# Arbol-Project/dcdf

Hardware: AMD Instinct MI355X
Metric: raster cells/s encoded (Snapshot+Log build) (higher is better)
Workload: dtype int32; 1 GPU; configs[2]: 4096x4096x365 i32 raster, seed 0xDCDF0003, tiled into 3072 [<=32,256,256] chunks; 3072 of them on this GPU; workload_key=config2/i32/n3072/w1, chunks_total=3072, chunks_on_rank0=3072, cells_total=6123683840, k=2, device=gfx950:sramecc+:xnack- AMD Radeon Graphics, 256 CUs, failed_tiles_rank0=0, encoded_bytes_rank0=4115239087, snapshots_rank0=3072, bytes_verified_vs_oracle=0, parallelism=chunks sharded over 1 GPU(s), no data-path collective

## Files before the change

dcdf_amd/csrc/k2r_encode.h:

```cpp
#pragma once
#include "k2r_exec.h"


#ifndef K2R_DIAG_SKIP
#define K2R_DIAG_SKIP 0
#endif

namespace k2r {

template <int LOG2S>
struct EncCfg {
    static_assert(LOG2S >= 3 && LOG2S <= 8, "kernel body written for sidelen 8..256 (the library dispatches 16..256)");
    static constexpr int H = LOG2S;
    static constexpr int S = 1 << LOG2S;
    static constexpr int NBLK = 1 << (2 * (LOG2S - 3));
    static constexpr int NT = NBLK;
    static constexpr int NW = NT < 64 ? 1 : NT / 64;
    static constexpr int NTOP = ((1 << (2 * (H - 2))) - 1) / 3;
    static constexpr int NTOPX = NTOP - (1 << (2 * (H - 3)));
    static constexpr int TBW = (NTOPX + 31) / 32 + 1;
    static constexpr int MAXV = ((1 << (2 * (H + 1))) - 1) / 3;
    static constexpr int MAXT = ((1 << (2 * H)) - 1) / 3;
    static constexpr int WV = (MAXV + 31) / 32;
    static constexpr int WT = (MAXT + 31) / 32;
// ... 205 lines not shown
            const uint32_t ob = o << 3;
            const ll2 a = *(__attribute__((address_space(1))) const ll2*)((gptr)ib + ob);
            const ll2 b = *(__attribute__((address_space(1))) const ll2*)((gptr)ib + ob + 16);
            x[0] = a.x; x[1] = a.y; x[2] = b.x; x[3] = b.y;
#else
            for (int i = 0; i < 4; i++) x[i] = ib[o + i];
#endif
            if (VEC == 4) {
                const double f[4] = {as_f64(x[0]), as_f64(x[1]), as_f64(x[2]), as_f64(x[3])};
                int32_t v[4];
                fixed4_f64(f, ta, (double)((int64_t)1 << ta.fbits), v, err);
#pragma unroll
                for (int dc = 0; dc < 4; dc++) dst[cell_m(dr, dc)] = v[dc];
            } else {
#pragma unroll
                for (int dc = 0; dc < 4; dc++) {
                    bad |= (uint32_t)(((uint64_t)x[dc] + (uint64_t)VALUE_LIMIT) >> 31 != 0);
                    dst[cell_m(dr, dc)] = (int32_t)x[dc];
                }
            }
        }
        if (bad && err == 0) err = ERR_RANGE;
    } else if (VEC) {
        const int32_t* ib = (const int32_t*)ta.base + (int64_t)inst * ta.st;
        const uint32_t o0 = rj * (uint32_t)ta.sr + cj;
#pragma unroll
        for (int dr = 0; dr < 4; dr++) {
            const uint32_t o = o0 + (uint32_t)dr * (uint32_t)ta.sr;
            int32_t v[4];
#if defined(__HIP_DEVICE_COMPILE__)
            typedef __attribute__((address_space(1))) const char* gptr;
            const uint32_t ob = o << 2;
#ifdef K2R_NT_LOADS
            typedef int i4v __attribute__((ext_vector_type(4)));
            const i4v av = __builtin_nontemporal_load((__attribute__((address_space(1))) const i4v*)((gptr)ib + ob));
            const int4 a = {av.x, av.y, av.z, av.w};
#else
            const int4 a = *(__attribute__((address_space(1))) const int4*)((gptr)ib + ob);
#endif
            v[0] = a.x; v[1] = a.y; v[2] = a.z; v[3] = a.w;
#else
            for (int i = 0; i < 4; i++) v[i] = ib[o + i];
#endif
            if (VEC == 2) {
                const float f[4] = {as_f32(v[0]), as_f32(v[1]), as_f32(v[2]), as_f32(v[3])};
                fixed4_f32(f, ta, (float)((int64_t)1 << ta.fbits), v, err);
            }
#pragma unroll
            for (int dc = 0; dc < 4; dc++) dst[cell_m(dr, dc)] = v[dc];
        }
    } else {
#pragma unroll
        for (int m = 0; m < 16; m++) {
            uint32_t r = rj + m_dr(m), c = cj + m_dc(m);
            if (PADDED) {
                r = r < ta.rows ? r : ta.rows - 1;
                c = c < ta.cols ? c : ta.cols - 1;
            }
            int64_t off = (int64_t)inst * ta.st + (int64_t)r * ta.sr + (int64_t)c * ta.sc;
            dst[m] = narrow(load_stored(ta, off, err), err);
        }
    }
}

template <class C>
K2R_HD uint32_t compact_slot(int tid, int j) {
    return 4u * (uint32_t)tid + (uint32_t)j;
}
template <class C>
K2R_HD void load_compact_raw(const uint32_t* scmp, int tid, int j, uint32_t (&w)[8]) {
    const uint32_t* p = scmp + (size_t)compact_slot<C>(tid, j) * 8;
#if defined(__HIP_DEVICE_COMPILE__)
    typedef __attribute__((address_space(1))) const char* gptr;
    const uint32_t ob = compact_slot<C>(tid, j) * 32u;
    const uint4 a = *(__attribute__((address_space(1))) const uint4*)((gptr)scmp + ob);
    const uint4 b = *(__attribute__((address_space(1))) const uint4*)((gptr)scmp + ob + 16);
    (void)p;
    w[0] = a.x; w[1] = a.y; w[2] = a.z; w[3] = a.w;
    w[4] = b.x; w[5] = b.y; w[6] = b.z; w[7] = b.w;
#else
    for (int i = 0; i < 8; i++) w[i] = p[i];
#endif
}
template <class C>
K2R_HD void load_compact(const uint32_t* scmp, int tid, int j, int32_t base, int32_t (&dst)[16]) {
    uint32_t w[8];
    load_compact_raw<C>(scmp, tid, j, w);
#pragma unroll
    for (int p = 0; p < 2; p++)
#pragma unroll
        for (int c = 0; c < 4; c++) {
            dst[8 * p + c] = base + (int32_t)(w[4 * p + c] & 0xffffu);
            dst[8 * p + 4 + c] = base + (int32_t)(w[4 * p + c] >> 16);
        }
}
template <class C>
K2R_HD void store_compact(uint32_t* scmp, int tid, int j, int32_t base, const int32_t (&src)[16]) {
    uint32_t* p = scmp + (size_t)compact_slot<C>(tid, j) * 8;
    uint32_t w[8];
#pragma unroll
    for (int q = 0; q < 2; q++)
#pragma unroll
        for (int c = 0; c < 4; c++) w[4 * q + c] = (uint32_t)(src[8 * q + c] - base) | ((uint32_t)(src[8 * q + 4 + c] - base) << 16);
#if defined(__HIP_DEVICE_COMPILE__)
    *(__attribute__((address_space(1))) uint4*)p = uint4{w[0], w[1], w[2], w[3]};
    *(__attribute__((address_space(1))) uint4*)(p + 4) = uint4{w[4], w[5], w[6], w[7]};
#else
    for (int i = 0; i < 8; i++) p[i] = w[i];
#endif
}
K2R_HD uint32_t pk_min_u16(uint32_t a, uint32_t b) {
#if defined(__HIP_DEVICE_COMPILE__)
    typedef unsigned short u16x2 __attribute__((ext_vector_type(2)));
    return __builtin_bit_cast(uint32_t, __builtin_elementwise_min(__builtin_bit_cast(u16x2, a), __builtin_bit_cast(u16x2, b)));
#else
    const uint32_t lo = (a & 0xffffu) < (b & 0xffffu) ? (a & 0xffffu) : (b & 0xffffu), hi = (a >> 16) < (b >> 16) ? (a >> 16) : (b >> 16);
    return lo | (hi << 16);
#endif
}
K2R_HD uint32_t pk_max_u16(uint32_t a, uint32_t b) {
#if defined(__HIP_DEVICE_COMPILE__)
    typedef unsigned short u16x2 __attribute__((ext_vector_type(2)));
    return __builtin_bit_cast(uint32_t, __builtin_elementwise_max(__builtin_bit_cast(u16x2, a), __builtin_bit_cast(u16x2, b)));
#else
    const uint32_t lo = (a & 0xffffu) > (b & 0xffffu) ? (a & 0xffffu) : (b & 0xffffu), hi = (a >> 16) > (b >> 16) ? (a >> 16) : (b >> 16);
    return lo | (hi << 16);
#endif
}
K2R_HD uint32_t nz(uint32_t v) {
#if defined(__HIP_DEVICE_COMPILE__)
    uint32_t r;
    asm("v_min_u32 %0, 1, %1" : "=v"(r) : "v"(v));
    return r;
#else
    return v != 0 ? 1u : 0u;
#endif
}
K2R_HD uint32_t mul24(uint32_t a, uint32_t b) {
#if defined(__HIP_DEVICE_COMPILE__)
    return __umul24(a, b);
#else
    return a * b;
#endif
}
K2R_HD uint32_t pk_lo16(uint32_t lo, uint32_t hi) {
#if defined(__HIP_DEVICE_COMPILE__)
    return __builtin_amdgcn_perm(hi, lo, 0x05040100u);
#else
    return (lo & 0xffffu) | (hi << 16);
#endif
}

K2R_HD uint32_t opaque(uint32_t v) {
#if defined(__HIP_DEVICE_COMPILE__)
    asm volatile("" : "+v"(v));
#endif
    return v;
}

K2R_HD void sched_fence() {
#if defined(__HIP_DEVICE_COMPILE__) && !defined(K2R_NO_SCHED_FENCE)
    __builtin_amdgcn_sched_barrier(0);
#endif
}

template <bool PADDED, int VEC>
K2R_HD void load_quad(const TileArgs& ta, uint32_t inst, uint32_t rq, uint32_t cq, int32_t (&dst)[4], int32_t& err) {
    if (VEC == 3 || VEC == 4) {
        const int64_t* ib = (const int64_t*)ta.base + (int64_t)inst * ta.st;
        const uint32_t o0 = rq * (uint32_t)ta.sr + cq;
        uint32_t bad = 0;
        int64_t raw[4];
#pragma unroll
        for (int dr = 0; dr < 2; dr++) {
            const uint32_t o = o0 + (uint32_t)dr * (uint32_t)ta.sr;
            int64_t x0, x1;
#if defined(__HIP_DEVICE_COMPILE__)
            typedef __attribute__((address_space(1))) const char* gptr;
            typedef long long ll2 __attribute__((ext_vector_type(2)));
            const ll2 a = *(__attribute__((address_space(1))) const ll2*)((gptr)ib + (o << 3));
            x0 = a.x; x1 = a.y;
#else
            x0 = ib[o]; x1 = ib[o + 1];
#endif
            raw[2 * dr] = x0;
            raw[2 * dr + 1] = x1;
        }
        if (VEC == 4) {
            const double f[4] = {as_f64(raw[0]), as_f64(raw[1]), as_f64(raw[2]), as_f64(raw[3])};
            fixed4_f64(f, ta, (double)((int64_t)1 << ta.fbits), dst, err);
        } else {
#pragma unroll
// ... 1296 lines not shown
        auto log_vmin = [&](int h, uint32_t j) -> int32_t {
            const int a = C::top_off(h) + (int)j;
            return sh.tmin[a] - sh.smin[a];
        };

        auto top_decode = [&](uint32_t n, int& h, uint32_t& j) {
            h = 4;
#pragma unroll
            for (int k = 4; k < H; k++)
                if (n >= (uint32_t)(C::top_off(k + 1) - C::NBLK)) h = k + 1;
            j = n - (uint32_t)(C::top_off(h) - C::NBLK);
        };
        auto tbit = [&](int h, uint32_t j) -> uint32_t { return (uint32_t)(C::top_off(h) - C::NBLK) + j; };

        ex.par_nosync([&](int tid, EncRegs& r) {
            uint32_t sI3 = 0, lI3 = 0;
            uint32_t wide = (r.flags >> 28) & 1u;
            Cls lMax, lMin;
            uint32_t sTop = 0, lTop = 0;
            auto node = [&](int h, uint32_t j) {
                if (PS(h, j)) {
                    if (h == 3) sI3 = 1;
                    else {
                        ex.lds_or(&sh.tbS[tbit(h, j) >> 5], 1u << (tbit(h, j) & 31));
                        sTop += (uint32_t)packTop(h);
                    }
                }
                if (have_s) {
                    const bool visL = (h == H) ? true : PL(h + 1, j >> 2);
                    const bool pL = PL(h, j);
                    const int32_t vx = log_vmax(h, j), vn = log_vmin(h, j);
                    lMax.add1(vx, visL);
                    lMin.add1(vn, pL);
                    wide |= ((visL && (vx < -32768 || vx > 32767)) || (pL && (vn < -32768 || vn > 32767))) ? 1u : 0u;
                    if (pL) {
                        if (h == 3) lI3 = 1;
                        else {
                            ex.lds_or(&sh.tbL[tbit(h, j) >> 5], 1u << (tbit(h, j) & 31));
                            lTop += (uint32_t)packTop(h);
                        }
                    }
                }
            };
            const uint32_t wt = opaque((uint32_t)tid);
            node(3, wt);
            if (tid == 0) {
                sh.stI = 0;
                sh.stQ = 0;
            }
            if (wt < (uint32_t)C::NTOPX) {
                int h;
                uint32_t j;
                top_decode(wt, h, j);
                node(h, j);
            }
            r.sc[1] = sI3 | (lI3 << 16);
            r.sc[2] = sTop;
            r.sc[4] = lTop;
            r.sc[5] = lMax.c1 | (lMin.c1 << 16);
            r.sc[6] = wide;
            uint32_t cL0 = 0, cL1 = 0, mL1 = 0, cL2 = 0, mL2 = 0;
            if (have_s) {
                const uint32_t fl = sh.li[tid];
                cL0 = popc32(sh.lq[tid][0]) + popc32(sh.lq[tid][1]);
                cL1 = popc32(fl & 0x0f0f0f0fu);
                mL1 = popc32(fl & 0xf0f0f0f0u);
#pragma unroll
                for (int j = 0; j < 4; j++) {
                    const int32_t vx = rec16(r.d2[j] & 0xffffu), vn = rec16(r.d2[j] >> 16);
                    r.d2[j] = ((uint32_t)vx & 0xffffu) | ((uint32_t)vn << 16);
                    const bool P2L = ((r.u2 >> j) & 1u) == 0 && ((r.flags >> j) & 1u) == 0;
                    cL2 += lI3 ? lng(vx) : 0u;
                    mL2 += P2L ? lng(vn) : 0u;
                }
            }
            r.sc[7] = cL0;
            r.sc[8] = cL1 | (cL2 << 16);
            r.sc[9] = mL1 | (mL2 << 16);
        });
        ex.stamp(2);
        ex.template scan_begin<10>();
        ex.stamp(3);

        auto classes_pass = [&](const int which) {
#ifdef K2R_SIM_TRACE
            if (EX::kSim) __builtin_printf("classes_pass(%d) inst=%u\n", which, inst);
#endif
            ex.par_nosync([&](int tid, EncRegs& r) {
                uint32_t r0, c0;
                blk_origin(tid, r0, c0);
                int32_t lerr = 0;
                Cls vMax, vMin;
                auto cnode = [&](int h, uint32_t j) {
                    if (which == 0) {
                        vMax.add(zz32(snap_vmax(h, j)), (h == H) ? true : PS(h + 1, j >> 2));
                        vMin.add(zz32(snap_vmin(h, j)), PS(h, j));
                    } else {
                        vMax.add(zz32(log_vmax(h, j)), (h == H) ? true : PL(h + 1, j >> 2));
                        vMin.add(zz32(log_vmin(h, j)), PL(h, j));
                    }
                };
                cnode(3, (uint32_t)tid);
                if (tid < C::NTOPX) {
                    int h;
                    uint32_t j;
                    top_decode((uint32_t)tid, h, j);
                    cnode(h, j);
                }
                const int32_t mn3 = sh.tmin[tid], mx3 = sh.tmax[tid];
                const bool inv3 = inval(r0, c0);
                const bool P3 = !inv3 && mn3 != mx3 && (which == 0 || sh.eq[tid] == 0);
#pragma unroll 1
                for (int j = 0; j < 4; j++) {
                    const uint32_t rj = r0 + 4 * (j >> 1), cj = c0 + 4 * (j & 1);
                    const bool inv2 = inval(rj, cj);
                    int32_t t16[16], s16[16];
                    load_sub16<PADDED, VEC>(ta, inst, r0, c0, j, t16, lerr);
                    if (which != 0) load_sub16<PADDED, VEC>(ta, s_idx, r0, c0, j, s16, lerr);
                    int32_t mn2 = t16[0], mx2 = t16[0], smn2 = 0, smx2 = 0;
#pragma unroll
                    for (int i = 1; i < 16; i++) {
                        mn2 = t16[i] < mn2 ? t16[i] : mn2;
                        mx2 = t16[i] > mx2 ? t16[i] : mx2;
                    }
                    if (which != 0) {
                        smn2 = smx2 = s16[0];
#pragma unroll
                        for (int i = 1; i < 16; i++) {
                            smn2 = s16[i] < smn2 ? s16[i] : smn2;
                            smx2 = s16[i] > smx2 ? s16[i] : smx2;
                        }
                    }
                    const bool unif2 = inv2 || mn2 == mx2;
                    bool P2;
                    if (which == 0) {
                        P2 = !unif2;
                        vMax.add(zz32(inv2 ? mx3 : mx3 - mx2), P3);
                        vMin.add(zz32(mn2 - mn3), P2);
                    } else {
                        P2 = !unif2 && ((r.flags >> j) & 1u) == 0;
                        vMax.add(zz32(inv2 ? 0 : mx2 - smx2), P3);
                        vMin.add(zz32(mn2 - smn2), P2);
                    }
                    if (!P2) continue;
#pragma unroll
                    for (int qq = 0; qq < 4; qq++) {
                        const uint32_t rq = rj + 2 * (qq >> 1), cq = cj + 2 * (qq & 1);
                        const bool inv1 = inval(rq, cq);
                        const int32_t mn1 = min4(t16[4 * qq], t16[4 * qq + 1], t16[4 * qq + 2], t16[4 * qq + 3]);
                        const int32_t mx1 = max4(t16[4 * qq], t16[4 * qq + 1], t16[4 * qq + 2], t16[4 * qq + 3]);
                        const bool unif1 = inv1 || mn1 == mx1;
                        if (which == 0) {
                            vMax.add(zz32(inv1 ? mx2 : mx2 - mx1), true);
                            vMin.add(zz32(mn1 - mn2), !unif1);
#pragma unroll
                            for (int i = 0; i < 4; i++)
                                vMax.add(zz32(inval(rq + (i >> 1), cq + (i & 1)) ? mx1 : mx1 - t16[4 * qq + i]), !unif1);
                        } else {
                            int32_t d[4];
#pragma unroll
                            for (int i = 0; i < 4; i++)
                                d[i] = inval(rq + (i >> 1), cq + (i & 1)) ? 0 : t16[4 * qq + i] - s16[4 * qq + i];
                            const int32_t smn1 = min4(s16[4 * qq], s16[4 * qq + 1], s16[4 * qq + 2], s16[4 * qq + 3]);
                            const int32_t smx1 = max4(s16[4 * qq], s16[4 * qq + 1], s16[4 * qq + 2], s16[4 * qq + 3]);
                            const bool P1 = !unif1 && !(d[0] == d[1] && d[0] == d[2] && d[0] == d[3]);
                            vMax.add(zz32(inv1 ? 0 : mx1 - smx1), true);
                            vMin.add(zz32(mn1 - smn1), P1);
#pragma unroll
                            for (int i = 0; i < 4; i++) vMax.add(zz32(d[i]), P1);
                        }
                    }
                }
                r.sc[10] = vMax.c1;
                r.sc[11] = vMax.c2;
                r.sc[12] = vMax.c3;
                r.sc[13] = vMin.c1;
                r.sc[14] = vMin.c2;
                r.sc[15] = vMin.c3;
            });
            ex.template reduce<6, 10>();
        };

        const bool cap254 = have_s && (blk_count - 1 == 254);
        auto plan = [&](const int stage) {
            ex.par([&](int tid, EncRegs&) {
                uint32_t T10[10];
                if (stage == 1) {
                    ex.template scan_finish<10>(T10);
                    for (uint32_t w = (uint32_t)tid; w <= (uint32_t)C::WT; w += NT) {
                        sh.bmT[w] = 0;
                        sh.bmE[w] = 0;
                        sh.bmM[0][w] = 0;
                    }
                    for (uint32_t w = (uint32_t)tid; w <= (uint32_t)C::WV; w += NT) sh.bmV0[w] = 0;
                }
                constexpr bool kTwoLanes = !EX::kSim && NT >= 2;
                if (tid >= (stage == 1 && kTwoLanes ? 2 : 1)) return;
                auto& pl = sh.pl;
                auto choose = [&](bool snap, const Totals<C>& W, uint32_t size, uint32_t narrow) {
                    pl.as_snapshot = snap ? 1u : 0u;
                    pl.isize = size;
                    pl.use_stash = (!snap && narrow && 5u * stI + 3u * stQ <= stash_cap && stI == W.Ni[2] && stQ == W.Ni[1]) ? 1u : 0u;
                    uint32_t rr = 0;
#pragma unroll
                    for (int h = 4; h <= H; h++) {
                        sh.ttR[h] = rr;
                        rr += W.Ni[h];
                    }
                    sh.ttR[H + 1] = rr;
                };
                if (stage == 1) {
                    const uint32_t t0 = T10[0], t1 = T10[1], t2 = T10[2], t3 = T10[3], t4 = T10[4], t5 = T10[5], t6 = T10[6], t7 = T10[7],
                                   t8 = T10[8], t9 = T10[9];
                    const uint32_t narrow = (have_s && t6 == 0) ? 1u : 0u;
                    const uint32_t lv2 = t5 & 0xffffu, lv1 = lv2 + (t8 >> 16), lv0 = lv1 + (t8 & 0xffffu);
                    const uint32_t lm2 = t5 >> 16, lm1 = lm2 + (t9 >> 16);
                    auto cand = [&](uint32_t c, Totals<C>& T, DacLayout& V, DacLayout& M, uint32_t& eo) {
                        T.from(c == 0 ? ((uint64_t)t0 | ((uint64_t)(t1 & 0xffffu) << 30)) : ((uint64_t)t3 | ((uint64_t)(t1 >> 16) << 30)),
                               c == 0 ? t2 : t4);
                        eo = 13 + bitmap_size(T.LT);
                        const uint32_t vbase = c == 0 ? eo : eo + bitmap_size(T.LT - T.M0);
                        const bool counts = c == 1 && narrow;
                        V = dac_layout(vbase, T.N0, counts ? lv0 + t7 : 0u, 0, 0);
                        M = dac_layout(V.end, T.M0, counts ? lm1 + (t9 & 0xffffu) : 0u, 0, 0);
                    };
                    uint32_t snap_lb, log_size, eq_off;
                    Totals<C> TW;
                    bool i_hold_log;
                    if (kTwoLanes) {
                        DacLayout V, M;
                        uint32_t eo;
                        cand((uint32_t)tid, TW, V, M, eo);
                        if (tid == 0 || have_s) {
                            pl.T[tid] = TW;
                            pl.V[tid] = V;
                            pl.M[tid] = M;
                        }
                        snap_lb = ex.lane_value(M.end, 0);
                        log_size = have_s ? ex.lane_value(M.end, 1) : 0u;
                        eq_off = have_s ? ex.lane_value(eo, 1) : 0u;
                        i_hold_log = tid == 1;
                    } else {
                        Totals<C> TS;
                        DacLayout SV, SM, LV{}, LM{};
                        uint32_t eo0, eo1 = 0;
                        cand(0, TS, SV, SM, eo0);
                        pl.T[0] = TS;
                        pl.V[0] = SV;
                        pl.M[0] = SM;
                        if (have_s) {
                            cand(1, TW, LV, LM, eo1);
                            pl.T[1] = TW;
                            pl.V[1] = LV;
                            pl.M[1] = LM;
                        }
                        snap_lb = SM.end;
                        log_size = have_s ? LM.end : 0u;
                        eq_off = eo1;
                        i_hold_log = true;
                    }
                    uint32_t need = 0;
                    if (have_s && !narrow) {
                        need = 1;
                        log_size = 0;
                    } else if (!have_s || cap254 || snap_lb <= log_size) {
                        need = 2;
                    } else if (i_hold_log) {
                        choose(false, TW, log_size, narrow);
                    }
                    if (tid == 0) {
                        pl.lngV[0] = lv0;
                        pl.lngV[1] = lv1;
                        pl.lngV[2] = lv2;
                        pl.lngM[1] = lm1;
                        pl.lngM[2] = lm2;
                        pl.narrow = narrow;
                        pl.log_size = log_size;
                        pl.eq_off = eq_off;
                        pl.snap_lb = snap_lb;
                        pl.need = need;
                    }
                } else if (stage == 2) {
                    pl.V[1] = dac_layout(pl.eq_off + bitmap_size(pl.T[1].LT - pl.T[1].M0), pl.T[1].N0, sh.tot[10], sh.tot[11], sh.tot[12]);
                    pl.M[1] = dac_layout(pl.V[1].end, pl.T[1].M0, sh.tot[13], sh.tot[14], sh.tot[15]);
                    pl.log_size = pl.M[1].end;
                    if (cap254 || pl.snap_lb <= pl.log_size) pl.need = 2;
                    else {
                        choose(false, pl.T[1], pl.log_size, pl.narrow);
                        pl.need = 0;
                    }
                } else {
                    const uint32_t sbase = 13 + bitmap_size(pl.T[0].LT);
                    pl.V[0] = dac_layout(sbase, pl.T[0].N0, sh.tot[10], sh.tot[11], sh.tot[12]);
                    pl.M[0] = dac_layout(pl.V[0].end, pl.T[0].M0, sh.tot[13], sh.tot[14], sh.tot[15]);
                    const bool snap = !have_s || cap254 || pl.M[0].end <= pl.log_size;
                    choose(snap, pl.T[snap ? 0 : 1], snap ? pl.M[0].end : pl.log_size, pl.narrow);
                    pl.need = 0;
                }
            });
        };
        plan(1);
        uint32_t need = ex.uni(sh.pl.need);
        if (need & 1u) {
            classes_pass(1);
            plan(2);
            need = ex.uni(sh.pl.need);
        }
        if (need & 2u) {
            classes_pass(0);
            plan(3);
        }
        const bool as_snapshot = ex.uni(sh.pl.as_snapshot) != 0;
        const bool use_stash = ex.uni(sh.pl.use_stash) != 0;
        const uint32_t isize = ex.uni(sh.pl.isize);
        const uint32_t log_eq_off = ex.uni(sh.pl.eq_off);
        const Totals<C>& TT = sh.pl.T[as_snapshot ? 0 : 1];
        const DacLayout& DV = sh.pl.V[as_snapshot ? 0 : 1];
        const DacLayout& DM = sh.pl.M[as_snapshot ? 0 : 1];

        uint32_t hdr_patch_off = 0, hdr_patch_val = 0;
        bool do_patch = false;
        if (as_snapshot) {
            if (have_s) {
                if (blk_hdr == NO_HDR) carry = blk_count;
                else {
                    do_patch = true;
                    hdr_patch_off = blk_hdr;
                    hdr_patch_val = blk_count;
                }
                n_blocks++;
            }
            blk_hdr = off;
            off += 1;
            blk_count = 0;
            s_idx = inst;
            n_snap++;
            const int32_t rmin = ex.uni(sh.tmin[C::top_off(H)]), rmax = ex.uni(sh.tmax[C::top_off(H)]);
            s_cmp = (int64_t)rmax - (int64_t)rmin <= 65535 && inst + 1 < ta.instants;
            s_base = rmin;
            cmp = (head && inst == 0) ? ta.shared_cmp : scmp;
        } else {
            n_log++;
        }
        if ((uint64_t)off + isize > cap) {
            status = ST_OUT_CAPACITY;
            break;
        }
        uint8_t* const io = out + off;
        n_stash += use_stash ? 1u : 0u;
        ex.stamp(12);
        ex.par([&](int tid, EncRegs& r) {
            const uint32_t pI12 = as_snapshot ? r.sc[0] : r.sc[3];
            const uint32_t pI3 = as_snapshot ? (r.sc[1] & 0xffffu) : (r.sc[1] >> 16);
            const uint32_t pL0 = r.sc[7], pL12 = r.sc[8], pM12 = r.sc[9];
            r.pf_lo = (uint64_t)pI12 | ((uint64_t)pI3 << 30);
            r.pf_l2 = (pL12 >> 16) | (pM12 & 0xffff0000u);
            sh.pfx[0][tid] = pI12;
            sh.pfx[1][tid] = pL0;
            sh.pfx[2][tid] = (pL12 & 0xffffu) | (pM12 << 16);
            if (tid <= C::TBW) {
                const uint32_t* const tbw = as_snapshot ? sh.tbS : sh.tbL;
                uint32_t run = 0;
                for (int w = 0; w < tid && w < C::TBW; w++) run += popc32(tbw[w]);
                sh.tbP[tid] = run;
            }
            if (tid == 0) {
                sh.nlistV = 0;
                sh.nlistM = 0;
                if (do_patch) out[hdr_patch_off] = (uint8_t)hdr_patch_val;
                io[0] = 2;
                store_be32(io + 1, ta.rows);
                store_be32(io + 5, ta.cols);
                store_be32(io + 9, (uint32_t)C::S);
                io[DV.bm_off[0] - 1] = (uint8_t)DV.nlev;
                io[DM.bm_off[0] - 1] = (uint8_t)DM.nlev;
                if (ta.minmax) {
                    ta.minmax[2 * inst] = sh.tmin[C::top_off(H)];
                    ta.minmax[2 * inst + 1] = sh.tmax[C::top_off(H)];
                }
            }
        });

        ex.stamp(4);
        const uint32_t nlevV = ex.uni(DV.nlev), nlevM = ex.uni(DM.nlev);
        const DacSink sinkV{io + ex.uni(DV.by_off[0]), sh.bmV0, listV, &sh.nlistV, ex.uni(DV.n[0]), ex.uni(DV.n[1]), inst, kGuardVPos,
                            io + ex.uni(DV.by_off[1]), use_stash ? sh.prefTopV : sh.prefV()};
        const DacSink sinkM{io + ex.uni(DM.by_off[0]), sh.bmM[0], listM, &sh.nlistM, ex.uni(DM.n[0]), ex.uni(DM.n[1]), inst, kGuardMPos,
                            io + ex.uni(DM.by_off[1]), sh.prefM};

        auto passA = [&](auto mode_tag) {
          constexpr int MODE = decltype(mode_tag)::value;
          ex.par_nosync([&](int tid, EncRegs& r) {
            uint32_t r0, c0;
            blk_origin(tid, r0, c0);
            const uint64_t pLo = r.pf_lo;

            const uint32_t* const tb = as_snapshot ? sh.tbS : sh.tbL;
            if (MODE == EM_P0) r.pa[2] = 0;
            constexpr int GMODE = (MODE == EM_P0) ? (int)EM_ONE : MODE;
            auto enode = [&](int h, uint32_t j, const int slot) {
                const bool vis = (h == H) ? true : bit_test(tb, tbit(h + 1, j >> 2));
                if (!vis) return;
                const bool p = (h == 3) ? (as_snapshot ? PS(3, j) : PL(3, j)) : bit_test(tb, tbit(h, j));
                auto trank = [&](uint32_t b) -> uint32_t {
                    return sh.tbP[b >> 5] + popc32(tb[b >> 5] & ((1u << (b & 31u)) - 1u));
                };
                uint32_t vrank = 0;
                if (h < H) vrank = 4 * (trank(tbit(h + 1, j >> 2)) - sh.ttR[h + 1]) + (j & 3);
                const uint32_t idx = TT.offV[h] + vrank;
                const uint32_t irank = (h == 3) ? unpackI(3, pLo, 0) : trank(tbit(h, j)) - sh.ttR[h];
                const uint32_t zv = zz32(as_snapshot ? snap_vmax(h, j) : log_vmax(h, j));
                emit_val<0, MODE>(ex, sinkV, idx, zv, tid);
                if (MODE == EM_P0) {
                    r.pa[3 * slot] = idx;
                    r.pa[2] |= (zv >> 8) << (16 * slot);
                }
                if (p) {
                    bm_set(ex, sh.bmT, guard_pos(ex, idx, 1, TT.LT, kGuardTOwn));
                    const uint32_t zm = zz32(as_snapshot ? snap_vmin(h, j) : log_vmin(h, j));
                    emit_val<1, MODE>(ex, sinkM, TT.offI[h] + irank, zm, tid);
                    if (MODE == EM_P0) {
                        r.pa[3 * slot + 1] = TT.offI[h] + irank;
                        r.pa[2] |= (zm >> 8) << (16 * slot + 8);
                    }
                } else if (!as_snapshot) {
                    const int a = C::top_off(h) + (int)j;
                    const bool e = !top_inval(h, j) && sh.tmin[a] != sh.tmax[a];
                    if (e) bm_set(ex, sh.bmE, guard_pos(ex, TT.offZ[h] + vrank - irank, 1, TT.LT - TT.M0, kGuardEOwn));
                }
            };
            const uint32_t wt = opaque((uint32_t)tid);
            enode(3, wt, 0);
            if (wt < (uint32_t)C::NTOPX) {
                int h;
                uint32_t j;
                top_decode(wt, h, j);
                enode(h, j, 1);
            }

            const int32_t mn3 = sh.tmin[tid], mx3 = sh.tmax[tid];
            const bool inv3 = inval(r0, c0);
            const uint32_t E1 = unpackI(1, pLo, 0), E2 = unpackI(2, pLo, 0), E3 = unpackI(3, pLo, 0);
            const bool P3 = !inv3 && mn3 != mx3 && (as_snapshot || sh.eq[tid] == 0);
            if (P3) {
                const uint32_t p2 = TT.offV[2] + 4 * E3;
                uint32_t tb2 = 0, z2v[4], zm2[4], erun = 0, elen = 0;
                bool P2[4];
#pragma unroll
                for (int j = 0; j < 4; j++) {
                    const bool inv2 = inval(r0 + 4 * (j >> 1), c0 + 4 * (j & 1));
                    const bool unif2 = ((r.u2 >> j) & 1u) != 0;
                    int32_t vx, vn;
                    if (MODE == EM_LIST) {
                        int32_t lerr = 0, t16[16];
                        load_sub16<PADDED, VEC>(ta, inst, r0, c0, j, t16, lerr);
                        int32_t mn2 = t16[0], mx2 = t16[0];
#pragma unroll
                        for (int i = 1; i < 16; i++) {
                            mn2 = t16[i] < mn2 ? t16[i] : mn2;
                            mx2 = t16[i] > mx2 ? t16[i] : mx2;
                        }
                        if (as_snapshot) {
                            vx = inv2 ? mx3 : mx3 - mx2;
                            vn = mn2 - mn3;
                        } else {
                            int32_t s16[16];
                            load_sub16<PADDED, VEC>(ta, s_idx, r0, c0, j, s16, lerr);
                            int32_t smn2 = s16[0], smx2 = s16[0];
#pragma unroll
                            for (int i = 1; i < 16; i++) {
                                smn2 = s16[i] < smn2 ? s16[i] : smn2;
                                smx2 = s16[i] > smx2 ? s16[i] : smx2;
                            }
                            vx = inv2 ? 0 : mx2 - smx2;
                            vn = mn2 - smn2;
                        }
                    } else {
                        vx = (int32_t)(int16_t)(r.d2[j] & 0xffffu);
                        vn = (int32_t)r.d2[j] >> 16;
                    }
                    if (as_snapshot) {
                        P2[j] = !unif2;
                        z2v[j] = zz32(vx);
                        zm2[j] = zz32(vn);
                    } else {
                        P2[j] = !unif2 && ((r.flags >> j) & 1u) == 0;
                        z2v[j] = zz32(vx);
                        zm2[j] = zz32(vn);
                        if (!P2[j]) {
                            erun = (erun << 1) | (unif2 ? 0u : 1u);
                            elen++;
                        }
                    }
                    tb2 = (tb2 << 1) | (P2[j] ? 1u : 0u);
                }
                emit4<0, GMODE>(ex, sinkV, p2, z2v[0], z2v[1], z2v[2], z2v[3], tid, sh.pl.lngV[2] + (r.pf_l2 & 0xffffu));
                bm_or_run(ex, sh.bmT, guard_pos(ex, p2, 4, TT.LT, kGuardTRun2), 4, tb2);
                if (!as_snapshot) bm_or_run(ex, sh.bmE, guard_pos<false>(ex, TT.offZ[2] + 4 * E3 - E2, elen, TT.LT - TT.M0, kGuardE2), elen, erun);
                uint32_t n2 = 0, pre = E1, lm = sh.pl.lngM[2] + (r.pf_l2 >> 16);
                const uint32_t cshift = as_snapshot ? 4u : 16u;
#pragma unroll
                for (int j = 0; j < 4; j++) {
                    if (P2[j]) {
                        emit_val<1, GMODE>(ex, sinkM, TT.offI[2] + E2 + n2, zm2[j], tid, lm);
                        lm += zm2[j] > 0xffu ? 1u : 0u;
                        if (MODE == EM_LIST)
                            sh.L2()[guard_pos(ex, E2 + n2, 1, 4 * C::NBLK, kGuardList2)] = ((uint32_t)tid << 2) | (uint32_t)j | (pre << 12);
                        n2++;
                        pre += (r.flags >> (cshift + 3 * j)) & 7u;
                    }
                }
            }
            guard_flush(ex);
        });
        };
        const uint32_t nI2 = ex.uni(TT.Ni[2]), nI1 = ex.uni(TT.Ni[1]);
        if (use_stash) {
            if (!(K2R_DIAG_SKIP & 1)) passA(EmTag<EM_P0>{});
            ex.stamp(10);
            auto passI = [&](auto ovf_tag) {
              constexpr bool OVF = decltype(ovf_tag)::value != 0;
              ex.par_nosync([&](int tid, EncRegs&) {
                const uint32_t offV1 = TT.offV[1], offZ1 = TT.offZ[1], offI1 = TT.offI[1], lt = TT.LT, ne = TT.LT - TT.M0;
                const uint32_t lv1 = sh.pl.lngV[1], lm1 = sh.pl.lngM[1];
                for (uint32_t k = (uint32_t)tid; k < nI2; k += NT) {
                    uint32_t rec[5];
                    if (!OVF || k < (uint32_t)SH::CAPI_REC) {
#pragma unroll
                        for (int i = 0; i < 5; i++) rec[i] = sh.pool[5u * k + i];
                    } else {
                        gload_words<5>(ovI + 5u * (k - (uint32_t)SH::CAPI_REC), rec);
                    }
                    const uint32_t hdr = rec[0];
                    const uint32_t own = hdr & 1023u;
                    const uint32_t pf = sh.pfx[0][own], pl = sh.pfx[2][own];
                    const uint32_t kk = ((pf >> 16) & 0x3fffu) + ((hdr >> 10) & 3u);
                    const uint32_t pre = (pf & 0xffffu) + ((hdr >> 12) & 15u);
                    const uint32_t tb1 = (hdr >> 16) & 15u, e4 = (hdr >> 20) & 15u, elen = 4u - popc32(tb1);
// ... 9 lines not shown
                    for (int qq = 0; qq < 4; qq++) w[qq] = rec[1 + qq];
                    const uint32_t p1 = offV1 + 4 * kk;
                    emit4<0, EM_ONE>(ex, sinkV, p1, zz32(rec16(w[0] & 0xffffu)), zz32(rec16(w[1] & 0xffffu)),
                                     zz32(rec16(w[2] & 0xffffu)), zz32(rec16(w[3] & 0xffffu)), tid,
                                     lv1 + (pl & 0xffffu) + popc32(below & 0x0f0f0f0fu));
                    bm_or_run(ex, sh.bmT, guard_pos(ex, p1, 4, lt, kGuardTRun1), 4, tb1);
                    bm_or_run(ex, sh.bmE, guard_pos<false>(ex, offZ1 + 4 * kk - pre, elen, ne, kGuardE1), elen, erun);
                    uint32_t n1 = 0, lm = lm1 + (pl >> 16) + popc32(below & 0xf0f0f0f0u);
#pragma unroll
                    for (int qq = 0; qq < 4; qq++) {
                        if ((tb1 >> (3 - qq)) & 1u) {
                            const uint32_t zm = zz32(rec16(w[qq] >> 16));
                            emit_val<1, EM_ONE>(ex, sinkM, offI1 + pre + n1, zm, tid, lm);
                            lm += zm > 0xffu ? 1u : 0u;
                            n1++;
                        }
                    }
                }
                guard_flush(ex);
              });
            };
            if (K2R_DIAG_SKIP & 2) {
            } else if (rec_ovf) passI(EmTag<1>{});
            else passI(EmTag<0>{});
            ex.stamp(11);
            auto passQ = [&](auto ovf_tag) {
              constexpr bool OVF = decltype(ovf_tag)::value != 0;
              ex.par([&](int tid, EncRegs&) {
                const uint32_t offV0 = TT.offV[0], lv0 = sh.pl.lngV[0];
                for (uint32_t m = (uint32_t)tid; m < nI1; m += NT) {
                    uint32_t q[3];
                    if (!OVF || m < (uint32_t)SH::CAPQ_REC) {
#pragma unroll
                        for (int i = 0; i < 3; i++) q[i] = sh.pool[SH::QBASE + 3u * m + i];
                    } else {
                        gload_words<3>(ovQ + 3u * (m - (uint32_t)SH::CAPQ_REC), q);
                    }
                    const uint32_t hdr = q[0], a = q[1], b = q[2];
                    const uint32_t own = hdr & 1023u;
                    const uint32_t ord = (hdr >> 10) & 15u;
                    const uint32_t pos = (sh.pfx[0][own] & 0xffffu) + ord;
                    const uint32_t f0 = sh.lq[own][0], f1 = sh.lq[own][1], cut = (1u << (4u * (ord & 7u))) - 1u;
                    const uint32_t before = ord < 8u ? popc32(f0 & cut) : popc32(f0) + popc32(f1 & cut);
                    emit4<0, EM_ONE>(ex, sinkV, offV0 + 4 * pos, zz32(rec16(a & 0xffffu)), zz32(rec16(a >> 16)),
                                     zz32(rec16(b & 0xffffu)), zz32(rec16(b >> 16)), tid, lv0 + sh.pfx[1][own] + before);
                }
                guard_flush(ex);
              });
            };
            if (K2R_DIAG_SKIP & 4) ex.barrier();
            else if (rec_ovf) passQ(EmTag<1>{});
            else passQ(EmTag<0>{});
            ex.stamp(6);
            {
                const uint32_t lt = ex.uni(TT.LT), m0 = ex.uni(TT.M0);
                const BmJob jobs[4] = {{sh.bmT, lt, nullptr, 0, io + 13},
                                       {sh.bmE, lt - m0, nullptr, 0, io + log_eq_off},
                                       {sh.bmV0, sinkV.n0, sh.prefTopV, SH::PREFTOP, nlevV > 0 ? io + ex.uni(DV.bm_off[0]) : nullptr},
                                       {sh.bmM[0], sinkM.n0, sh.prefM, SH::PREFTOP, nlevM > 0 ? io + ex.uni(DM.bm_off[0]) : nullptr}};
                if (!(K2R_DIAG_SKIP & 8)) bitmaps_finish<C, 4>(ex, jobs);
            }
            ex.stamp(8);
            if (nlevV > 1 || nlevM > 1) {
                if (!(K2R_DIAG_SKIP & 16)) ex.par_nosync([&](int tid, EncRegs& r) {
                    auto put = [&](const DacSink& d, uint32_t* bm0, uint32_t pos, uint32_t hi) {
                        if (hi) {
                            pos = guard_pos(ex, pos, 1, d.n0 < 32u * SH::PREFTOP ? d.n0 : 32u * SH::PREFTOP, d.code);
                            gstore8(d.plane1 + guard_pos(ex, bm_rank(bm0, d.pref, pos), 1, d.n1, d.code + 1), (uint8_t)hi);
                        }
                    };
                    const uint32_t hb = r.pa[2];
                    put(sinkV, sh.bmV0, r.pa[0], hb & 0xffu);
                    put(sinkM, sh.bmM[0], r.pa[1], (hb >> 8) & 0xffu);
                    put(sinkV, sh.bmV0, r.pa[3], (hb >> 16) & 0xffu);
                    put(sinkM, sh.bmM[0], r.pa[4], hb >> 24);
                    guard_flush(ex);
                });
                ex.stamp(14);
                if (nlevV > 1 && !(K2R_DIAG_SKIP & 32)) bitmap_write_zero<C>(ex, sinkV.n1, io + ex.uni(DV.bm_off[1]));
                if (nlevM > 1 && !(K2R_DIAG_SKIP & 32)) bitmap_write_zero<C>(ex, sinkM.n1, io + ex.uni(DM.bm_off[1]));
            }
            ex.stamp(9);
        } else {
            if (as_snapshot && s_cmp) compact_pass(inst, head && inst == 0);
            if (head && inst == 0) {
                ex.publish(ta.shared_flag, s_cmp ? PART_CMP : PART_NOCMP, (uint32_t)s_base);
                published = true;
            }
            passA(EmTag<EM_LIST>{});
            ex.barrier();
            ex.stamp(10);
            ex.par([&](int tid, EncRegs&) {
                int32_t lerr = 0;
                for (uint32_t k = (uint32_t)tid; k < nI2; k += NT) {
                    const uint32_t ent = sh.L2()[k];
                    const uint32_t blk = (ent >> 2) & (C::NBLK - 1), j = ent & 3u, pre = ent >> 12;
                    uint32_t r0, c0;
                    blk_origin((int)blk, r0, c0);
                    const uint32_t rj = r0 + 4 * (j >> 1), cj = c0 + 4 * (j & 1);
                    int32_t t16[16];
                    load_sub16<PADDED, VEC>(ta, inst, r0, c0, (int)j, t16, lerr);
                    int32_t mn1[4], mx1[4];
                    bool inv1[4];
#pragma unroll
                    for (int qq = 0; qq < 4; qq++) {
                        mn1[qq] = min4(t16[4 * qq], t16[4 * qq + 1], t16[4 * qq + 2], t16[4 * qq + 3]);
                        mx1[qq] = max4(t16[4 * qq], t16[4 * qq + 1], t16[4 * qq + 2], t16[4 * qq + 3]);
                        inv1[qq] = inval(rj + 2 * (qq >> 1), cj + 2 * (qq & 1));
                    }
                    uint32_t z1v[4], zm1[4], tb1 = 0, erun = 0, elen = 0;
                    bool P1[4];
                    if (as_snapshot) {
                        const int32_t mn2 = min4(mn1[0], mn1[1], mn1[2], mn1[3]);
                        const int32_t mx2 = max4(mx1[0], mx1[1], mx1[2], mx1[3]);
#pragma unroll
                        for (int qq = 0; qq < 4; qq++) {
                            P1[qq] = !inv1[qq] && mn1[qq] != mx1[qq];
                            z1v[qq] = zz32(inv1[qq] ? mx2 : mx2 - mx1[qq]);
                            zm1[qq] = zz32(mn1[qq] - mn2);
                            tb1 = (tb1 << 1) | (P1[qq] ? 1u : 0u);
                        }
                    } else {
                        int32_t s16[16];
                        load_sub16<PADDED, VEC>(ta, s_idx, r0, c0, (int)j, s16, lerr);
#pragma unroll
                        for (int qq = 0; qq < 4; qq++) {
                            const uint32_t rq = rj + 2 * (qq >> 1), cq = cj + 2 * (qq & 1);
                            int32_t d[4];
#pragma unroll
                            for (int i = 0; i < 4; i++)
                                d[i] = inval(rq + (i >> 1), cq + (i & 1)) ? 0 : t16[4 * qq + i] - s16[4 * qq + i];
                            const int32_t smn1 = min4(s16[4 * qq], s16[4 * qq + 1], s16[4 * qq + 2], s16[4 * qq + 3]);
                            const int32_t smx1 = max4(s16[4 * qq], s16[4 * qq + 1], s16[4 * qq + 2], s16[4 * qq + 3]);
                            const bool eq1 = d[0] == d[1] && d[0] == d[2] && d[0] == d[3];
                            const bool unif1 = inv1[qq] || mn1[qq] == mx1[qq];
                            P1[qq] = !unif1 && !eq1;
                            z1v[qq] = zz32(inv1[qq] ? 0 : mx1[qq] - smx1);
                            zm1[qq] = zz32(mn1[qq] - smn1);
                            tb1 = (tb1 << 1) | (P1[qq] ? 1u : 0u);
                            if (!P1[qq]) {
                                erun = (erun << 1) | (unif1 ? 0u : 1u);
                                elen++;
                            }
                        }
                    }
                    const uint32_t p1 = TT.offV[1] + 4 * k;
                    emit4<0>(ex, sinkV, p1, z1v[0], z1v[1], z1v[2], z1v[3], tid);
                    bm_or_run(ex, sh.bmT, guard_pos(ex, p1, 4, TT.LT, kGuardTRun1), 4, tb1);
                    if (!as_snapshot) bm_or_run(ex, sh.bmE, guard_pos<false>(ex, TT.offZ[1] + 4 * k - pre, elen, TT.LT - TT.M0, kGuardE1), elen, erun);
                    uint32_t n1 = 0;
#pragma unroll
                    for (int qq = 0; qq < 4; qq++) {
                        if (P1[qq]) {
                            emit_val<1>(ex, sinkM, TT.offI[1] + pre + n1, zm1[qq], tid);
                            sh.L1()[guard_pos(ex, pre + n1, 1, 16 * C::NBLK, kGuardList1)] = (uint16_t)((blk << 4) | (j << 2) | (uint32_t)qq);
                            n1++;
                        }
                    }
                }
                guard_flush(ex);
            });

            ex.stamp(11);
            ex.par([&](int tid, EncRegs&) {
                int32_t lerr = 0;
                constexpr uint32_t U = 4;
                for (uint32_t m0 = (uint32_t)tid; m0 < nI1; m0 += U * NT) {
                    int32_t t4[U][4], s4[U][4];
                    uint32_t rq[U], cq[U];
#pragma unroll
                    for (uint32_t u = 0; u < U; u++) {
                        const uint32_t m = m0 + u * NT;
                        if (m >= nI1) continue;
                        const uint32_t key = sh.L1()[m];
                        const uint32_t blk = key >> 4, j = (key >> 2) & 3u, qq = key & 3u;
                        uint32_t r0, c0;
                        blk_origin((int)blk, r0, c0);
                        rq[u] = r0 + 4 * (j >> 1) + 2 * (qq >> 1);
                        cq[u] = c0 + 4 * (j & 1) + 2 * (qq & 1);
                        load_quad<PADDED, VEC>(ta, inst, rq[u], cq[u], t4[u], lerr);
                        if (!as_snapshot) load_quad<PADDED, VEC>(ta, s_idx, rq[u], cq[u], s4[u], lerr);
                    }
#pragma unroll
                    for (uint32_t u = 0; u < U; u++) {
                        const uint32_t m = m0 + u * NT;
                        if (m >= nI1) continue;
                        uint32_t z[4];
                        if (as_snapshot) {
                            const int32_t mx1 = max4(t4[u][0], t4[u][1], t4[u][2], t4[u][3]);
#pragma unroll
                            for (int i = 0; i < 4; i++) z[i] = zz32(inval(rq[u] + (i >> 1), cq[u] + (i & 1)) ? mx1 : mx1 - t4[u][i]);
                        } else {
#pragma unroll
                            for (int i = 0; i < 4; i++) z[i] = zz32(inval(rq[u] + (i >> 1), cq[u] + (i & 1)) ? 0 : t4[u][i] - s4[u][i]);
                        }
                        emit4<0>(ex, sinkV, TT.offV[0] + 4 * m, z[0], z[1], z[2], z[3], tid);
                    }
                }
                guard_flush(ex);
            });
            ex.stamp(as_snapshot ? 5 : 6);
            bitmap_finish_write<C>(ex, sh.bmT, ex.uni(TT.LT), sh.prefM, io + 13);
            if (!as_snapshot) bitmap_finish_write<C>(ex, sh.bmE, ex.uni(TT.LT) - ex.uni(TT.M0), sh.prefM, io + log_eq_off);
            ex.stamp(7);
            auto uni_layout = [&](const DacLayout& L) {
                DacLayout U;
#pragma unroll
                for (int i = 0; i < 5; i++) U.n[i] = ex.uni(L.n[i]);
#pragma unroll
                for (int i = 0; i < 4; i++) {
                    U.bm_off[i] = ex.uni(L.bm_off[i]);
                    U.by_off[i] = ex.uni(L.by_off[i]);
                }
                U.nlev = ex.uni(L.nlev);
                U.end = ex.uni(L.end);
                return U;
            };
            dac_finish<C>(ex, uni_layout(DV), io, sh.bmV0, sh.bmV1(), sh.prefV(), listV, &sh.nlistV);
            ex.stamp(8);
            dac_finish<C>(ex, uni_layout(DM), io, sh.bmM[0], sh.bmM[1], sh.prefM, listM, &sh.nlistM);
            ex.stamp(9);
        }

        off += isize;
        blk_count++;
    }

    if (head && !published) ex.publish(ta.shared_flag, PART_FAILED, 0u);

    ex.par([&](int tid, EncRegs&) {
        if (tid == 0) {
            if (status == ST_OK) {
                if (blk_hdr == NO_HDR) carry = blk_count;
                else out[blk_hdr] = (uint8_t)blk_count;
                if (!cont) store_be32(out + 2, n_blocks + 1);
            }
            res->carry_count = carry;
            const bool faulted = sh.fault[0] != 0;
            res->status = faulted ? (int32_t)ST_INTERNAL : status;
            res->snapshots = n_snap;
            res->logs = n_log;
            res->stash_logs = n_stash;
            res->len = (status == ST_OK && !faulted) ? off : 0;
            for (int i = 0; i < 6; i++) res->dbg[i] = sh.fault[i];
            for (int i = 0; i < NPROF; i++) res->prof[i] = sh.prof[i];
        }
#ifdef K2R_PROFILE
        if (!EX::kSim && (tid & 63) == 0)
            for (int k = 0; k < NPROF; k++) {
                res->pw[tid >> 6][k][0] = sh.pw[tid >> 6][k][0];
                res->pw[tid >> 6][k][1] = sh.pw[tid >> 6][k][1];
            }
#endif
    });
}

}
```

Baseline: 547.6 billion cells/s.

## Fuse compact snapshot copy into classes pass and read compact tiles downstream

When the snapshot range fits in 16 bits, the snapshot classes pass now writes the 16-bit compact copy of each tile as it loads it, which removes the separate compact_pass. The later snapshot emit stages (level-2 min/max, level-1 list and leaf values) then read the half-size compact buffer instead of reloading full int32 raster data. This cuts global memory traffic in exchange for a global barrier after the store and extra code paths that must handle padding and base offsets correctly.

```diff
diff --git a/dcdf_amd/csrc/k2r_encode.h b/dcdf_amd/csrc/k2r_encode.h
--- a/dcdf_amd/csrc/k2r_encode.h
+++ b/dcdf_amd/csrc/k2r_encode.h
@@ -311,17 +311,36 @@
     for (int i = 0; i < 8; i++) w[i] = p[i];
 #endif
 }
+K2R_HD void unpack_compact(const uint32_t (&w)[8], int32_t base, int32_t (&dst)[16]) {
+#pragma unroll
+    for (int p = 0; p < 2; p++)
+#pragma unroll
+        for (int c = 0; c < 4; c++) {
+            dst[8 * p + c] = base + (int32_t)(w[4 * p + c] & 0xffffu);
+            dst[8 * p + 4 + c] = base + (int32_t)(w[4 * p + c] >> 16);
+        }
+}
+template <class C>
+K2R_HD void load_compact_quad(const uint32_t* scmp, int tid, int j, uint32_t qq, int32_t (&dst)[4]) {
+    uint32_t w[4];
+#if defined(__HIP_DEVICE_COMPILE__)
+    typedef __attribute__((address_space(1))) const char* gptr;
+    const uint32_t ob = compact_slot<C>(tid, j) * 32u + (qq >> 1) * 16u;
+    const uint4 a = *(__attribute__((address_space(1))) const uint4*)((gptr)scmp + ob);
+    w[0] = a.x; w[1] = a.y; w[2] = a.z; w[3] = a.w;
+#else
+    const uint32_t* p = scmp + (size_t)compact_slot<C>(tid, j) * 8 + 4 * (qq >> 1);
+    for (int i = 0; i < 4; i++) w[i] = p[i];
+#endif
+    const uint32_t s = 16u * (qq & 1u);
+#pragma unroll
+    for (int c = 0; c < 4; c++) dst[c] = (int32_t)((w[c] >> s) & 0xffffu);
+}
 template <class C>
 K2R_HD void load_compact(const uint32_t* scmp, int tid, int j, int32_t base, int32_t (&dst)[16]) {
     uint32_t w[8];
     load_compact_raw<C>(scmp, tid, j, w);
-#pragma unroll
-    for (int p = 0; p < 2; p++)
-#pragma unroll
-        for (int c = 0; c < 4; c++) {
-            dst[8 * p + c] = base + (int32_t)(w[4 * p + c] & 0xffffu);
-            dst[8 * p + 4 + c] = base + (int32_t)(w[4 * p + c] >> 16);
-        }
+    unpack_compact(w, base, dst);
 }
 template <class C>
 K2R_HD void store_compact(uint32_t* scmp, int tid, int j, int32_t base, const int32_t (&src)[16]) {
@@ -1799,7 +1818,7 @@
         ex.template scan_begin<10>();
         ex.stamp(3);
 
-        auto classes_pass = [&](const int which) {
+        auto classes_pass = [&](const int which, const bool store) {
 #ifdef K2R_SIM_TRACE
             if (EX::kSim) __builtin_printf("classes_pass(%d) inst=%u\n", which, inst);
 #endif
@@ -1834,6 +1853,7 @@
                     int32_t t16[16], s16[16];
                     load_sub16<PADDED, VEC>(ta, inst, r0, c0, j, t16, lerr);
                     if (which != 0) load_sub16<PADDED, VEC>(ta, s_idx, r0, c0, j, s16, lerr);
+                    if (store) store_compact<C>(cmp, tid, j, s_base, t16);
                     int32_t mn2 = t16[0], mx2 = t16[0], smn2 = 0, smx2 = 0;
 #pragma unroll
                     for (int i = 1; i < 16; i++) {
@@ -1895,6 +1915,7 @@
                 r.sc[14] = vMin.c2;
                 r.sc[15] = vMin.c3;
             });
+            if (store) ex.barrier_global();
             ex.template reduce<6, 10>();
         };
 
@@ -2019,12 +2040,22 @@
         plan(1);
         uint32_t need = ex.uni(sh.pl.need);
         if (need & 1u) {
-            classes_pass(1);
+            classes_pass(1, false);
             plan(2);
             need = ex.uni(sh.pl.need);
         }
+        bool copied = false;
         if (need & 2u) {
-            classes_pass(0);
+#ifndef K2R_AB_NO_FUSE
+            if (!have_s && !kRegCopy) {
+                const int32_t rmin = ex.uni(sh.tmin[C::top_off(H)]), rmax = ex.uni(sh.tmax[C::top_off(H)]);
+                s_cmp = (int64_t)rmax - (int64_t)rmin <= 65535 && inst + 1 < ta.instants;
+                s_base = rmin;
+                cmp = head ? ta.shared_cmp : scmp;
+                copied = s_cmp;
+            }
+#endif
+            classes_pass(0, copied);
             plan(3);
         }
         const bool as_snapshot = ex.uni(sh.pl.as_snapshot) != 0;
@@ -2065,6 +2096,11 @@
         }
         uint8_t* const io = out + off;
         n_stash += use_stash ? 1u : 0u;
+#ifndef K2R_AB_NO_COPYREAD
+        const bool snap_copy = !kRegCopy && as_snapshot && s_cmp;
+#else
+        const bool snap_copy = false;
+#endif
         ex.stamp(12);
         ex.par([&](int tid, EncRegs& r) {
             const uint32_t pI12 = as_snapshot ? r.sc[0] : r.sc[3];
@@ -2163,12 +2199,29 @@
                 const uint32_t p2 = TT.offV[2] + 4 * E3;
                 uint32_t tb2 = 0, z2v[4], zm2[4], erun = 0, elen = 0;
                 bool P2[4];
+                uint32_t cw[4][8];
+                if (MODE == EM_LIST && snap_copy) {
+#pragma unroll
+                    for (int j = 0; j < 4; j++) load_compact_raw<C>(cmp, tid, j, cw[j]);
+                }
 #pragma unroll
                 for (int j = 0; j < 4; j++) {
                     const bool inv2 = inval(r0 + 4 * (j >> 1), c0 + 4 * (j & 1));
                     const bool unif2 = ((r.u2 >> j) & 1u) != 0;
                     int32_t vx, vn;
-                    if (MODE == EM_LIST) {
+                    if (MODE == EM_LIST && snap_copy) {
+                        uint32_t lo = cw[j][0], hi = cw[j][0];
+#pragma unroll
+                        for (int i = 1; i < 8; i++) {
+                            lo = pk_min_u16(lo, cw[j][i]);
+                            hi = pk_max_u16(hi, cw[j][i]);
+                        }
+                        const uint32_t mn16 = (lo & 0xffffu) < (lo >> 16) ? (lo & 0xffffu) : (lo >> 16);
+                        const uint32_t mx16 = (hi & 0xffffu) > (hi >> 16) ? (hi & 0xffffu) : (hi >> 16);
+                        const int32_t mn2 = s_base + (int32_t)mn16, mx2 = s_base + (int32_t)mx16;
+                        vx = inv2 ? mx3 : mx3 - mx2;
+                        vn = mn2 - mn3;
+                    } else if (MODE == EM_LIST) {
                         int32_t lerr = 0, t16[16];
                         load_sub16<PADDED, VEC>(ta, inst, r0, c0, j, t16, lerr);
                         int32_t mn2 = t16[0], mx2 = t16[0];
@@ -2346,7 +2399,7 @@
             }
             ex.stamp(9);
         } else {
-            if (as_snapshot && s_cmp) compact_pass(inst, head && inst == 0);
+            if (as_snapshot && s_cmp && !copied) compact_pass(inst, head && inst == 0);
             if (head && inst == 0) {
                 ex.publish(ta.shared_flag, s_cmp ? PART_CMP : PART_NOCMP, (uint32_t)s_base);
                 published = true;
@@ -2354,7 +2407,59 @@
             passA(EmTag<EM_LIST>{});
             ex.barrier();
             ex.stamp(10);
-            ex.par([&](int tid, EncRegs&) {
+            if (snap_copy) ex.par([&](int tid, EncRegs&) {
+                constexpr uint32_t U = 4;
+                for (uint32_t k0 = (uint32_t)tid; k0 < nI2; k0 += U * NT) {
+                    uint32_t w[U][8], ent[U];
+#pragma unroll
+                    for (uint32_t u = 0; u < U; u++) {
+                        const uint32_t k = k0 + u * NT;
+                        if (k >= nI2) continue;
+                        ent[u] = sh.L2()[k];
+                        load_compact_raw<C>(cmp, (int)((ent[u] >> 2) & (C::NBLK - 1)), (int)(ent[u] & 3u), w[u]);
+                    }
+#pragma unroll
+                    for (uint32_t u = 0; u < U; u++) {
+                        const uint32_t k = k0 + u * NT;
+                        if (k >= nI2) continue;
+                        const uint32_t blk = (ent[u] >> 2) & (C::NBLK - 1), j = ent[u] & 3u, pre = ent[u] >> 12;
+                        uint32_t r0, c0;
+                        blk_origin((int)blk, r0, c0);
+                        const uint32_t rj = r0 + 4 * (j >> 1), cj = c0 + 4 * (j & 1);
+                        int32_t t16[16];
+                        unpack_compact(w[u], s_base, t16);
+                        int32_t mn1[4], mx1[4];
+                        bool inv1[4];
+#pragma unroll
+                        for (int qq = 0; qq < 4; qq++) {
+                            mn1[qq] = min4(t16[4 * qq], t16[4 * qq + 1], t16[4 * qq + 2], t16[4 * qq + 3]);
+                            mx1[qq] = max4(t16[4 * qq], t16[4 * qq + 1], t16[4 * qq + 2], t16[4 * qq + 3]);
+                            inv1[qq] = inval(rj + 2 * (qq >> 1), cj + 2 * (qq & 1));
+                        }
+                        const int32_t mn2 = min4(mn1[0], mn1[1], mn1[2], mn1[3]);
+                        const int32_t mx2 = max4(mx1[0], mx1[1], mx1[2], mx1[3]);
+                        uint32_t z1v[4], tb1 = 0, n1 = 0;
+#pragma unroll
+                        for (int qq = 0; qq < 4; qq++) {
+                            z1v[qq] = zz32(inv1[qq] ? mx2 : mx2 - mx1[qq]);
+                            tb1 = (tb1 << 1) | ((!inv1[qq] && mn1[qq] != mx1[qq]) ? 1u : 0u);
+                        }
+                        const uint32_t p1 = TT.offV[1] + 4 * k;
+                        emit4<0>(ex, sinkV, p1, z1v[0], z1v[1], z1v[2], z1v[3], tid);
+                        bm_or_run(ex, sh.bmT, guard_pos(ex, p1, 4, TT.LT, kGuardTRun1), 4, tb1);
+#pragma unroll
+                        for (int qq = 0; qq < 4; qq++) {
+                            if ((tb1 >> (3 - qq)) & 1u) {
+                                emit_val<1>(ex, sinkM, TT.offI[1] + pre + n1, zz32(mn1[qq] - mn2), tid);
+                                sh.L1()[guard_pos(ex, pre + n1, 1, 16 * C::NBLK, kGuardList1)] = (uint16_t)((blk << 4) | (j << 2) | (uint32_t)qq);
+                                n1++;
+                            }
+                        }
+                    }
+                }
+                guard_flush(ex);
+            });
+            else ex.par([&](int tid, EncRegs&) {
                 int32_t lerr = 0;
                 for (uint32_t k = (uint32_t)tid; k < nI2; k += NT) {
                     const uint32_t ent = sh.L2()[k];
@@ -2442,6 +2547,10 @@
                         blk_origin((int)blk, r0, c0);
                         rq[u] = r0 + 4 * (j >> 1) + 2 * (qq >> 1);
                         cq[u] = c0 + 4 * (j & 1) + 2 * (qq & 1);
+                        if (snap_copy) {
+                            load_compact_quad<C>(cmp, (int)blk, (int)j, qq, t4[u]);
+                            continue;
+                        }
                         load_quad<PADDED, VEC>(ta, inst, rq[u], cq[u], t4[u], lerr);
                         if (!as_snapshot) load_quad<PADDED, VEC>(ta, s_idx, rq[u], cq[u], s4[u], lerr);
                     }
@@ -2452,8 +2561,9 @@
                         uint32_t z[4];
                         if (as_snapshot) {
                             const int32_t mx1 = max4(t4[u][0], t4[u][1], t4[u][2], t4[u][3]);
-#pragma unroll
-                            for (int i = 0; i < 4; i++) z[i] = zz32(inval(rq[u] + (i >> 1), cq[u] + (i & 1)) ? mx1 : mx1 - t4[u][i]);
+                            const int32_t mx1abs = (PADDED && snap_copy) ? mx1 + s_base : mx1;
+#pragma unroll
+                            for (int i = 0; i < 4; i++) z[i] = zz32(inval(rq[u] + (i >> 1), cq[u] + (i & 1)) ? mx1abs : mx1 - t4[u][i]);
                         } else {
 #pragma unroll
                             for (int i = 0; i < 4; i++) z[i] = zz32(inval(rq[u] + (i >> 1), cq[u] + (i & 1)) ? 0 : t4[u][i] - s4[u][i]);
```

Result: no change. 543.3 billion cells/s (-0.8%).

## Build snapshot compact copy during classes pass and read it in emit passes

Applied to the files above, without the earlier changes.

When the root range fits in 16 bits, the classes pass now writes the 16-bit compact copy of each sub-block while it already holds the tile values, replacing the separate compact_pass with just a global barrier. The later snapshot emission passes (list, level-2 and level-1 quads) then read from the packed 16-bit compact buffer instead of reloading the full int32 raster. This is meant to cut global memory reads of the raw tile. In exchange the compact copy is stored speculatively, before the instant is known to become a snapshot, so the write is wasted when it turns out to be a log.

```diff
diff --git a/dcdf_amd/csrc/k2r_encode.h b/dcdf_amd/csrc/k2r_encode.h
--- a/dcdf_amd/csrc/k2r_encode.h
+++ b/dcdf_amd/csrc/k2r_encode.h
@@ -337,6 +337,21 @@
 #else
     for (int i = 0; i < 8; i++) p[i] = w[i];
 #endif
+}
+template <class C>
+K2R_HD void load_compact_quad(const uint32_t* scmp, uint32_t blk, uint32_t j, uint32_t qq, int32_t base, int32_t (&dst)[4]) {
+    const uint32_t wo = compact_slot<C>((int)blk, (int)j) * 8u + 4u * (qq >> 1);
+    uint32_t w[4];
+#if defined(__HIP_DEVICE_COMPILE__)
+    typedef __attribute__((address_space(1))) const char* gptr;
+    const uint4 a = *(__attribute__((address_space(1))) const uint4*)((gptr)scmp + wo * 4u);
+    w[0] = a.x; w[1] = a.y; w[2] = a.z; w[3] = a.w;
+#else
+    for (int i = 0; i < 4; i++) w[i] = scmp[wo + i];
+#endif
+    const uint32_t sh = 16u * (qq & 1u);
+#pragma unroll
+    for (int c = 0; c < 4; c++) dst[c] = base + (int32_t)((w[c] >> sh) & 0xffffu);
 }
 K2R_HD uint32_t pk_min_u16(uint32_t a, uint32_t b) {
 #if defined(__HIP_DEVICE_COMPILE__)
@@ -1799,6 +1814,9 @@
         ex.template scan_begin<10>();
         ex.stamp(3);
 
+        const int32_t root_min = ex.uni(sh.tmin[C::top_off(H)]), root_max = ex.uni(sh.tmax[C::top_off(H)]);
+        const bool pre_cmp = !have_s && !kRegCopy && inst + 1 < ta.instants && (int64_t)root_max - (int64_t)root_min <= 65535;
+        uint32_t* const pre_dst = (head && inst == 0) ? ta.shared_cmp : scmp;
         auto classes_pass = [&](const int which) {
 #ifdef K2R_SIM_TRACE
             if (EX::kSim) __builtin_printf("classes_pass(%d) inst=%u\n", which, inst);
@@ -1833,6 +1851,7 @@
                     const bool inv2 = inval(rj, cj);
                     int32_t t16[16], s16[16];
                     load_sub16<PADDED, VEC>(ta, inst, r0, c0, j, t16, lerr);
+                    if (which == 0 && pre_cmp) store_compact<C>(pre_dst, tid, j, root_min, t16);
                     if (which != 0) load_sub16<PADDED, VEC>(ta, s_idx, r0, c0, j, s16, lerr);
                     int32_t mn2 = t16[0], mx2 = t16[0], smn2 = 0, smx2 = 0;
 #pragma unroll
@@ -2065,6 +2084,7 @@
         }
         uint8_t* const io = out + off;
         n_stash += use_stash ? 1u : 0u;
+        const bool snap_copy = as_snapshot && s_cmp && !kRegCopy;
         ex.stamp(12);
         ex.par([&](int tid, EncRegs& r) {
             const uint32_t pI12 = as_snapshot ? r.sc[0] : r.sc[3];
@@ -2170,7 +2190,8 @@
                     int32_t vx, vn;
                     if (MODE == EM_LIST) {
                         int32_t lerr = 0, t16[16];
-                        load_sub16<PADDED, VEC>(ta, inst, r0, c0, j, t16, lerr);
+                        if (snap_copy) load_compact<C>(cmp, tid, j, s_base, t16);
+                        else load_sub16<PADDED, VEC>(ta, inst, r0, c0, j, t16, lerr);
                         int32_t mn2 = t16[0], mx2 = t16[0];
 #pragma unroll
                         for (int i = 1; i < 16; i++) {
@@ -2346,7 +2367,10 @@
             }
             ex.stamp(9);
         } else {
-            if (as_snapshot && s_cmp) compact_pass(inst, head && inst == 0);
+            if (as_snapshot && s_cmp) {
+                if (pre_cmp) ex.barrier_global();
+                else compact_pass(inst, head && inst == 0);
+            }
             if (head && inst == 0) {
                 ex.publish(ta.shared_flag, s_cmp ? PART_CMP : PART_NOCMP, (uint32_t)s_base);
                 published = true;
@@ -2363,7 +2387,8 @@
                     blk_origin((int)blk, r0, c0);
                     const uint32_t rj = r0 + 4 * (j >> 1), cj = c0 + 4 * (j & 1);
                     int32_t t16[16];
-                    load_sub16<PADDED, VEC>(ta, inst, r0, c0, (int)j, t16, lerr);
+                    if (snap_copy) load_compact<C>(cmp, (int)blk, (int)j, s_base, t16);
+                    else load_sub16<PADDED, VEC>(ta, inst, r0, c0, (int)j, t16, lerr);
                     int32_t mn1[4], mx1[4];
                     bool inv1[4];
 #pragma unroll
@@ -2442,7 +2467,8 @@
                         blk_origin((int)blk, r0, c0);
                         rq[u] = r0 + 4 * (j >> 1) + 2 * (qq >> 1);
                         cq[u] = c0 + 4 * (j & 1) + 2 * (qq & 1);
-                        load_quad<PADDED, VEC>(ta, inst, rq[u], cq[u], t4[u], lerr);
+                        if (snap_copy) load_compact_quad<C>(cmp, blk & (uint32_t)(C::NBLK - 1), j, qq, s_base, t4[u]);
+                        else load_quad<PADDED, VEC>(ta, inst, rq[u], cq[u], t4[u], lerr);
                         if (!as_snapshot) load_quad<PADDED, VEC>(ta, s_idx, rq[u], cq[u], s4[u], lerr);
                     }
 #pragma unroll
```

After: 547.9 billion cells/s before, 548.5 billion cells/s after (median of 6 runs). No clear change (+0.1%).
